# mfkiwl/msckf_stereo_c

Measured on AMD Instinct MI355X. Metric: stereo frames/sec/node on EuRoC-shape input; ATE RMSE vs CPU ref, higher is better.
Workload: dtype f64

## Files before the change

msckf_stereo_c_amd/csrc/hip/fe_kernels.hip:

```cpp
#include <stdlib.h>
#include <mutex>
#include "fe_device.h"

__device__ __forceinline__ int reflect101(int i, int n) {
    if (n == 1) return 0;
    while (i < 0 || i >= n) { i = (i < 0) ? -i : 2 * (n - 1) - i; }
    return i;
}

#define P3_TW 16
#define P3_TH 8
struct Pyr3Job { const uint8_t *src; uint8_t *d1, *d2, *d3; int w0, h0; };

namespace {
constexpr int P3_R2H = 2 * P3_TH + 4, P3_R1H = 2 * P3_R2H + 4, P3_R0H = 2 * P3_R1H + 4;
constexpr int P3_P2W = 2 * P3_TW + 8, P3_P1W = 2 * (2 * P3_TW + 4) + 8;
constexpr int P3_P1S = P3_P1W + 8, P3_P2S = P3_P2W + 8;
typedef uint32_t __attribute__((aligned(1))) pd_u32u;

__device__ __forceinline__ uint2 pd_h4(uint32_t w0, uint32_t w1, uint32_t w2) {
    const int b0 = w0 & 255u, b1 = (w0 >> 8) & 255u, b2 = (w0 >> 16) & 255u, b3 = w0 >> 24, b4 = w1 & 255u, b5 = (w1 >> 8) & 255u,
              b6 = (w1 >> 16) & 255u, b7 = w1 >> 24, b8 = w2 & 255u, b9 = (w2 >> 8) & 255u, b10 = (w2 >> 16) & 255u;
    const uint32_t h0 = (uint32_t)(b0 + 4 * b1 + 6 * b2 + 4 * b3 + b4), h1 = (uint32_t)(b2 + 4 * b3 + 6 * b4 + 4 * b5 + b6);
    const uint32_t h2 = (uint32_t)(b4 + 4 * b5 + 6 * b6 + 4 * b7 + b8), h3 = (uint32_t)(b6 + 4 * b7 + 6 * b8 + 4 * b9 + b10);
// ... 278 lines not shown
    DetPix l_mid = load(ys - 4), l_dn = load(ys - 3), l_nx = load(ys - 2);
    int cy = ys / ch, yin = ys - cy * ch;
    int bs[4] = {0, 0, 0, 0};
    unsigned long long bk[4] = {0ULL, 0ULL, 0ULL, 0ULL};
    const int n_rows = seg_rows;
#pragma unroll 1
    for (int k = 0; k < n_rows; ++k) {
        const int y = ys + k;
        const bool row_ok = y < y_end;
        const DetPix enx = load(pr + 3), lnx = load(y - 1);
        {
            int Ha[4], Hb[4], Hc[4];
            det_hrow(e_up, e_mid, e_dn.hi, Ha, Hb, Hc);
#pragma unroll
            for (int j = 0; j < 4; ++j) { Va[j] += Ha[j]; Vb[j] += Hb[j]; Vc[j] += Hc[j]; }
            e_up = e_mid.hi; e_mid = e_dn; e_dn = e_nx; e_nx = enx; ++pr;
        }
#pragma unroll
        for (int j = 0; j < 4; ++j) {
            if (!(col_ok[j] && row_ok)) continue;
            const int a = Va[j], b = Vb[j], d = Vc[j];
            const int X = (a + d) - max(det_floor, bs[j]);
            if (X <= 0) continue;
            const int df = a - d;
            if (abs(df) >= X || 2 * abs(b) >= X) continue;
            const double discd = (double)df * (double)df + 4.0 * ((double)b * (double)b);
            if (discd >= (double)X * (double)X) continue;
            const long long disc = (long long)df * df + 4LL * ((long long)b * b);
            const int score = (a + d) - (int)isqrt48((unsigned long long)disc, discd);
            bs[j] = score;
            bk[j] = det_key(gen, score, (unsigned int)(yin * cw + xin[j]));
        }
        {
            int Ha[4], Hb[4], Hc[4];
            det_hrow(l_up, l_mid, l_dn.hi, Ha, Hb, Hc);
#pragma unroll
            for (int j = 0; j < 4; ++j) { Va[j] -= Ha[j]; Vb[j] -= Hb[j]; Vc[j] -= Hc[j]; }
            l_up = l_mid.hi; l_mid = l_dn; l_dn = l_nx; l_nx = lnx;
        }
        ++yin;
        const bool flush = job_on && row_ok && (yin == ch || y + 1 == y_end);
        if (cw < 4) {
            if (flush) {
#pragma unroll
                for (int j = 0; j < 4; ++j) {
                    if (bk[j]) atomicMax(&cell_keys[cy * det_cols + cx[j]], bk[j]);
                    bs[j] = 0; bk[j] = 0ULL;
                }
            }
        } else if (__any(flush)) {
            unsigned long long ka = 0ULL, kb = 0ULL;
#pragma unroll
            for (int j = 0; j < 4; ++j) {
                const unsigned long long v = flush ? bk[j] : 0ULL;
                if (cx[j] == cx[0]) ka = v > ka ? v : ka; else kb = v > kb ? v : kb;
            }
            const bool two = cx[3] != cx[0];
#pragma unroll 1
            for (int pass = 0; pass < 2; ++pass) {
                unsigned long long kk = pass ? kb : ka;
                const int id = flush ? (pass ? (two ? cx[3] : -1 - r) : cx[0]) : -1 - r;
                if (pass && !__any(flush && two)) break;
                {
                    const int o = det_dpp0<0x101>(id + 0x40000000) - 0x40000000; const unsigned long long v = det_dpp0_64<0x101>(kk);
                    if (o == id && v > kk) kk = v;
                }
                {
                    const int o = det_dpp0<0x102>(id + 0x40000000) - 0x40000000; const unsigned long long v = det_dpp0_64<0x102>(kk);
                    if (o == id && v > kk) kk = v;
                }
                {
                    const int o = det_dpp0<0x104>(id + 0x40000000) - 0x40000000; const unsigned long long v = det_dpp0_64<0x104>(kk);
                    if (o == id && v > kk) kk = v;
                }
                {
                    const int o = det_dpp0<0x108>(id + 0x40000000) - 0x40000000; const unsigned long long v = det_dpp0_64<0x108>(kk);
                    if (o == id && v > kk) kk = v;
                }
                const int left = det_dpp0<0x111>(id + 0x40000000) - 0x40000000;
                if (id >= 0 && left != id && kk) atomicMax(&cell_keys[cy * det_cols + id], kk);
            }
            if (flush) {
#pragma unroll
                for (int j = 0; j < 4; ++j) { bs[j] = 0; bk[j] = 0ULL; }
            }
        }
        if (yin == ch) { yin = 0; ++cy; }
    }
}

extern "C" void fe_launch_detect(const FeStreamDev *streams_dev, int n_streams, int max_w, int max_h, unsigned int gen, hipStream_t st) {
    const int strips = (max_w - 2 * DET_BORDER + DS_COLS - 1) / DS_COLS, rows = max_h - 2 * DET_BORDER;
    if (strips <= 0 || rows <= 0) return;
    int seg_rows = 32;
    while (seg_rows < 128 && (long long)n_streams * strips * ((rows + seg_rows - 1) / seg_rows) / 4 > 32768) seg_rows *= 2;
    const int segs = (rows + seg_rows - 1) / seg_rows;
    const int waves = (strips * segs + 3) / 4;
    hipLaunchKernelGGL(k_detect_cells, dim3(8 * ((n_streams + 7) / 8) * waves), dim3(64), 0, st, streams_dev, n_streams, strips, seg_rows, waves, gen);
}


__device__ __forceinline__ double det_atan(double x) {
    const bool inv = x > 1.0;
    if (inv) x = 1.0 / x;
    double c = 0.0, ac = 0.0;
    if (x > 0.875)      { c = 1.0;  ac = 0.78539816339744830962; }
    else if (x > 0.625) { c = 0.75; ac = 0.64350110879328438680; }
    else if (x > 0.375) { c = 0.5;  ac = 0.46364760900080611621; }
    else if (x > 0.125) { c = 0.25; ac = 0.24497866312686415417; }
    const double z = (x - c) / (1.0 + x * c);
    const double z2 = z * z;
    double p = 1.0 / 21.0;
    p = 1.0 / 19.0 - z2 * p;
    p = 1.0 / 17.0 - z2 * p;
    p = 1.0 / 15.0 - z2 * p;
    p = 1.0 / 13.0 - z2 * p;
    p = 1.0 / 11.0 - z2 * p;
    p = 1.0 / 9.0 - z2 * p;
    p = 1.0 / 7.0 - z2 * p;
    p = 1.0 / 5.0 - z2 * p;
    p = 1.0 / 3.0 - z2 * p;
    p = 1.0 - z2 * p;
    const double a = ac + z * p;
    return inv ? 1.5707963267948966192 - a : a;
}
__device__ __forceinline__ double det_tan(double t) {
    const bool inv = t > 0.78539816339744830962;
    if (inv) t = 1.5707963267948966192 - t;
    const double t2 = t * t;
    double s = 1.0 / 121645100408832000.0;
    s = 1.0 / 355687428096000.0 - t2 * s;
    s = 1.0 / 1307674368000.0 - t2 * s;
    s = 1.0 / 6227020800.0 - t2 * s;
    s = 1.0 / 39916800.0 - t2 * s;
    s = 1.0 / 362880.0 - t2 * s;
    s = 1.0 / 5040.0 - t2 * s;
    s = 1.0 / 120.0 - t2 * s;
    s = 1.0 / 6.0 - t2 * s;
    s = t * (1.0 - t2 * s);
    double c = 1.0 / 6402373705728000.0;
    c = 1.0 / 20922789888000.0 - t2 * c;
    c = 1.0 / 87178291200.0 - t2 * c;
    c = 1.0 / 479001600.0 - t2 * c;
    c = 1.0 / 3628800.0 - t2 * c;
    c = 1.0 / 40320.0 - t2 * c;
    c = 1.0 / 720.0 - t2 * c;
    c = 1.0 / 24.0 - t2 * c;
    c = 0.5 - t2 * c;
    c = 1.0 - t2 * c;
    return inv ? c / s : s / c;
}


__device__ __forceinline__ void undistort_pt(const CamDev &cam, const double *R, float u, float v, float &xo, float &yo) {
    const double fx = cam.K[0], fy = cam.K[1], cx = cam.K[2], cy = cam.K[3];
    double x = ((double)u - cx) / fx, y = ((double)v - cy) / fy;
    if (cam.model == MSKF_MODEL_EQUIDISTANT) {
        const double *k = cam.D;
        double theta_d = sqrt(x * x + y * y);
        const double half_pi = 1.5707963267948966;
        theta_d = theta_d > half_pi ? half_pi : (theta_d < -half_pi ? -half_pi : theta_d);
        double scale = 0.0;
        if (theta_d > 1e-8) {
            double theta = theta_d;
            for (int j = 0; j < 10; ++j) {
                const double t2 = theta * theta, t4 = t2 * t2, t6 = t4 * t2, t8 = t6 * t2;
                const double k0t2 = k[0] * t2, k1t4 = k[1] * t4, k2t6 = k[2] * t6, k3t8 = k[3] * t8;
                const double fix = (theta * (1 + k0t2 + k1t4 + k2t6 + k3t8) - theta_d) /
                                   (1 + 3 * k0t2 + 5 * k1t4 + 7 * k2t6 + 9 * k3t8);
                theta = theta - fix;
                if (fabs(fix) < 1e-8) break;
            }
            scale = det_tan(theta) / theta_d;
        }
        x = x * scale; y = y * scale;
    } else {
        const double k1 = cam.D[0], k2 = cam.D[1], p1 = cam.D[2], p2 = cam.D[3];
        const double x0 = x, y0 = y;
        for (int j = 0; j < 5; ++j) {
            const double r2 = x * x + y * y;
            const double icdist = 1.0 / (1.0 + (k2 * r2 + k1) * r2);
            const double deltaX = 2.0 * p1 * x * y + p2 * (r2 + 2.0 * x * x);
            const double deltaY = p1 * (r2 + 2.0 * y * y) + 2.0 * p2 * x * y;
            x = (x0 - deltaX) * icdist;
            y = (y0 - deltaY) * icdist;
        }
    }
    if (R) {
        const double X = R[0] * x + R[1] * y + R[2];
        const double Y = R[3] * x + R[4] * y + R[5];
        const double Wd = R[6] * x + R[7] * y + R[8];
        x = X / Wd; y = Y / Wd;
    } else {
        x = x / 1.0; y = y / 1.0;
    }
    xo = (float)(x * 1.0 + 0.0);
    yo = (float)(y * 1.0 + 0.0);
}

__device__ __forceinline__ void distort_pt(const CamDev &cam, float xf, float yf, float &uo, float &vo) {
    const double fx = cam.K[0], fy = cam.K[1], cx = cam.K[2], cy = cam.K[3];
    const double x = (double)xf, y = (double)yf;
    double xd, yd;
    if (cam.model == MSKF_MODEL_EQUIDISTANT) {
        const double *k = cam.D;
        const double r = sqrt(x * x + y * y);
        const double theta = det_atan(r);
        const double t2 = theta * theta, t4 = t2 * t2, t6 = t4 * t2, t8 = t4 * t4;
        const double theta_d = theta * (1 + k[0] * t2 + k[1] * t4 + k[2] * t6 + k[3] * t8);
        const double scale = (r > 1e-8) ? theta_d / r : 1.0;
        xd = x * scale; yd = y * scale;
    } else {
        const double k1 = cam.D[0], k2 = cam.D[1], p1 = cam.D[2], p2 = cam.D[3];
        const double r2 = x * x + y * y, r4 = r2 * r2;
        const double a1 = 2.0 * x * y, a2 = r2 + 2.0 * x * x, a3 = r2 + 2.0 * y * y;
        const double cdist = 1.0 + k1 * r2 + k2 * r4;
        xd = x * cdist + p1 * a1 + p2 * a2;
        yd = y * cdist + p1 * a3 + p2 * a1;
    }
    uo = (float)(xd * fx + cx);
    vo = (float)(yd * fy + cy);
}

#define LK_HALF 7
#define LK_WIN 15
#define LK_ITERS 30

template <int CTRL> __device__ __forceinline__ int dpp_add(int v) {
    return v + __builtin_amdgcn_update_dpp(0, v, CTRL, 0xf, 0xf, false);
}
__device__ __forceinline__ double lk_scaled_f64(long long b) {
    return __longlong_as_double(b + 0x41F8000000000000LL) - 6442450944.0;
}

typedef short l4_v2s __attribute__((ext_vector_type(2)));
#define L4_DW 6
#define L4_TROWS 18
#define L4_SROWS 20
#define L4_MAXOX 8
#define L4_MAXOY (L4_SROWS - 16)

typedef unsigned short l4_v2u __attribute__((ext_vector_type(2)));
template <int KA, int KC> __device__ __forceinline__ int l4_mad24_k(int x) {
    int d;
    asm("v_mad_i32_i24 %0, %1, %2, %3" : "=v"(d) : "n"(KA), "v"(x), "n"(KC));
    return d;
}
template <int KA> __device__ __forceinline__ int l4_mad24_kv(int x, int c) {
    int d;
    asm("v_mad_i32_i24 %0, %1, %2, %3" : "=v"(d) : "n"(KA), "v"(x), "v"(c));
    return d;
}
__device__ __forceinline__ int l4_mad24(int a, int b, int c) {
    int d;
    asm("v_mad_i32_i24 %0, %1, %2, %3" : "=v"(d) : "v"(a), "v"(b), "s"(c));
    return d;
}
__device__ __forceinline__ int l4_mad24_vvv(int a, int b, int c) {
    int d;
    asm("v_mad_i32_i24 %0, %1, %2, %3" : "=v"(d) : "v"(a), "v"(b), "v"(c));
    return d;
}
__device__ __forceinline__ int l4_dot2(int pair, int w, int acc) {
    return __builtin_amdgcn_sdot2(__builtin_bit_cast(l4_v2s, pair), __builtin_bit_cast(l4_v2s, w), acc, false);
}
__device__ __forceinline__ int l4_dot2k(int pair, int w, int k) {
    return __builtin_amdgcn_sdot2(__builtin_bit_cast(l4_v2s, pair), __builtin_bit_cast(l4_v2s, w), k, true);
}
__device__ __forceinline__ int l4_pack_shr9(int a, int b) {
    const l4_v2u v = __builtin_bit_cast(l4_v2u, __builtin_amdgcn_perm((uint32_t)b, (uint32_t)a, 0x06050201u));
    return __builtin_bit_cast(int, (l4_v2u)(v >> (unsigned short)1));
}
#define L4_SHL1 0x101
#define L4_SHR1 0x111
template <int CTRL> __device__ __forceinline__ int l4_dpp0(int v) {
    return __builtin_amdgcn_update_dpp(0, v, CTRL, 0xf, 0xf, true);
}
__device__ __forceinline__ long long l4_row_sum(int v) {
    v = dpp_add<0xB1>(v);
    v = dpp_add<0x4E>(v);
    long long s = (long long)v;
    {
        const int lo = __builtin_amdgcn_update_dpp(0, (int)s, 0x141, 0xf, 0xf, true), hi = __builtin_amdgcn_update_dpp(0, (int)(s >> 32), 0x141, 0xf, 0xf, true);
        s += (long long)(((unsigned long long)(unsigned int)hi << 32) | (unsigned int)lo);
    }
    {
        const int lo = __builtin_amdgcn_update_dpp(0, (int)s, 0x140, 0xf, 0xf, true), hi = __builtin_amdgcn_update_dpp(0, (int)(s >> 32), 0x140, 0xf, 0xf, true);
        s += (long long)(((unsigned long long)(unsigned int)hi << 32) | (unsigned int)lo);
    }
    return s;
}

struct __attribute__((packed, aligned(4))) l4_u4 { uint32_t v[4]; };
struct __attribute__((packed, aligned(4))) l4_u2 { uint32_t v[2]; };
template <int ROWS>
__device__ __forceinline__ void l4_stage(const uint8_t *img, int w, int h, int x0, int y0, uint32_t *dst, int r, bool on) {
    const bool fast = x0 >= 0 && y0 >= 0 && x0 + 4 * L4_DW <= w && y0 + ROWS <= h;
    if (fast) {
        if (on) {
            const uint8_t *p = img + l4_mad24_vvv(y0 + r, w, x0);
            const l4_u4 a = *(const l4_u4 *)p;
            const l4_u2 b = *(const l4_u2 *)(p + 16);
            uint32_t *d = dst + L4_DW * r;
            d[0] = a.v[0]; d[1] = a.v[1]; d[2] = a.v[2]; d[3] = a.v[3]; d[4] = b.v[0]; d[5] = b.v[1];
            if (r < ROWS - 16) {
                const uint8_t *p2 = img + l4_mad24_vvv(y0 + 16 + r, w, x0);
                const l4_u4 a2 = *(const l4_u4 *)p2;
                const l4_u2 b2 = *(const l4_u2 *)(p2 + 16);
                uint32_t *d2 = dst + L4_DW * (16 + r);
                d2[0] = a2.v[0]; d2[1] = a2.v[1]; d2[2] = a2.v[2]; d2[3] = a2.v[3]; d2[4] = b2.v[0]; d2[5] = b2.v[1];
            }
        }
        return;
    }
    constexpr int N = ROWS * L4_DW, PER = (N + 15) / 16;
    typedef uint32_t __attribute__((aligned(1))) l4_u32u;
    uint32_t v[PER];
#pragma unroll
    for (int i = 0; i < PER; ++i) {
        const int e = r + 16 * i;
        v[i] = 0;
        if (on && e < N) {
            const int row = (e * 43) >> 8, c = e - L4_DW * row;
            const uint8_t *rp = img + l4_mad24_vvv(min(max(y0 + row, 0), h - 1), w, 0);
            const int xb = x0 + 4 * c, xc = min(max(xb, 0), w - 4), sh = xb - xc;
            const uint32_t D = *(const l4_u32u *)(rp + xc);
            const uint32_t first = (D & 255u) * 0x01010101u, last = (D >> 24) * 0x01010101u;
            v[i] = sh < 0 ? first : sh >= 4 ? last : __builtin_amdgcn_alignbyte(last, D, (uint32_t)sh);
        }
    }
#pragma unroll
    for (int i = 0; i < PER; ++i) { const int e = r + 16 * i; if (on && e < N) dst[e] = v[i]; }
}

template <int K> __device__ __forceinline__ int l4_pair(const uint32_t *a) {
    constexpr int q = K >> 2, m = K & 3;
    if (m == 0) return (int)__builtin_amdgcn_perm(0u, a[q], 0x0c010c00u);
    if (m == 1) return (int)__builtin_amdgcn_perm(0u, a[q], 0x0c020c01u);
    if (m == 2) return (int)__builtin_amdgcn_perm(0u, a[q], 0x0c030c02u);
    return (int)__builtin_amdgcn_perm(a[q + 1], a[q], 0x0c040c03u);
}
template <int N, int K = 0> struct L4Pairs {
    static __device__ __forceinline__ void run(const uint32_t *a, int *pr) { pr[K] = l4_pair<K>(a); L4Pairs<N, K + 1>::run(a, pr); }
};
template <int N> struct L4Pairs<N, N> { static __device__ __forceinline__ void run(const uint32_t *, int *) {} };

__device__ __forceinline__ void l4_weights(float fa, float fb, int &wtop, int &wbot) {
    const int qa = __float2int_rn(fa * 16384.0f), qb = __float2int_rn(fb * 16384.0f);
    const int w00 = l4_mad24(16384 - qa, 16384 - qb, 8192) >> 14;
    const int w01 = l4_mad24(qa, 16384 - qb, 8192) >> 14;
// ... 15 lines not shown
        const float sc = __int_as_float((127 - l) << 23);
        const float pwx = ax * sc - (float)LK_HALF, pwy = ay * sc - (float)LK_HALF;
        if (l == MSKF_LEVELS - 1) { ncx = bx * sc; ncy = by * sc; }
        else { ncx = ncx * 2.0f; ncy = ncy * 2.0f; }
        int ipx = (int)floorf(pwx), ipy = (int)floorf(pwy);
        bool lvl_on = alive && !(ipx < -LK_WIN || ipx >= aw || ipy < -LK_WIN || ipy >= ah);
        if (alive && !lvl_on && l == 0) status = 0;
        if (!lvl_on) { ipx = 0; ipy = 0; }
        int wtop, wbot;
        l4_weights(lvl_on ? pwx - (float)ipx : 0.f, lvl_on ? pwy - (float)ipy : 0.f, wtop, wbot);
        const int ax0 = (ipx - 1) & ~3, ay0 = ipy - 1, oxa = ipx - 1 - ax0;
        float wx = ncx - (float)LK_HALF, wy = ncy - (float)LK_HALF;
        int inx0 = (int)floorf(wx), iny0 = (int)floorf(wy);
        const bool in_b0 = !(inx0 < -LK_WIN || inx0 >= bw || iny0 < -LK_WIN || iny0 >= bh);
        if (!(lvl_on && in_b0)) { inx0 = 0; iny0 = 0; }
        int bx0 = (inx0 - 2) & ~3, by0 = iny0 - 2;
        __syncthreads();
        l4_stage<L4_TROWS>(imA, aw, ah, ax0, ay0, sT, r, true);
        l4_stage<L4_SROWS>(imB, bw, bh, bx0, by0, sS, r, true);
        __syncthreads();
        int V[17], E[17];
        {
            uint32_t d[6], a[5];
            int pr[17];
            const uint32_t *rp = sT + (r + 1) * L4_DW;
#pragma unroll
            for (int i = 0; i < 6; ++i) d[i] = rp[i];
#pragma unroll
            for (int i = 0; i < 5; ++i) a[i] = __builtin_amdgcn_alignbyte(d[i + 1], d[i], oxa);
            L4Pairs<17>::run(a, pr);
            int Bv[17];
#pragma unroll
            for (int c = 0; c < 17; ++c) { V[c] = l4_dot2k(pr[c], wtop, 256); Bv[c] = l4_dot2k(pr[c], wbot, 0); }
            const uint32_t *ep = sT + (r == 0 ? 0 : 17) * L4_DW;
#pragma unroll
            for (int i = 0; i < 6; ++i) d[i] = ep[i];
#pragma unroll
            for (int i = 0; i < 5; ++i) a[i] = __builtin_amdgcn_alignbyte(d[i + 1], d[i], oxa);
            L4Pairs<17>::run(a, pr);
            const int wsel = r == 0 ? wtop : wbot;
#pragma unroll
            for (int c = 0; c < 17; ++c) E[c] = l4_dot2(pr[c], wsel, r == 0 ? Bv[c] + 256 : V[c]) >> 9;
#pragma unroll
            for (int c = 0; c < 17; ++c) V[c] = (V[c] + l4_dpp0<L4_SHL1>(Bv[c])) >> 9;
            if (r == 15) {
#pragma unroll
                for (int c = 0; c < 17; ++c) V[c] = E[c];
            }
        }
        int Pp[8], Ixp[8], Iyp[8];
        int A11 = 0, A12 = 0, A22 = 0;
        {
            int f[17], e[17];
#pragma unroll
            for (int c = 0; c < 17; ++c) {
                const int up = __builtin_amdgcn_update_dpp(E[c], V[c], L4_SHR1, 0xf, 0xf, false);
                const int dn = l4_dpp0<L4_SHL1>(V[c]);
                f[c] = up + dn; e[c] = dn - up;
            }
            int gx[16], gy[16], pv[16];
#pragma unroll
            for (int i = 0; i < 15; ++i) {
                const int sx = l4_mad24_kv<10>(V[i + 2] - V[i], l4_mad24_k<3, 16>(f[i + 2] - f[i]));
                const int sy = l4_mad24_kv<10>(e[i + 1], l4_mad24_k<3, 16>(e[i] + e[i + 2]));
                gx[i] = sx >> 5;
                gy[i] = sy >> 5;
                pv[i] = V[i + 1];
            }
            gx[15] = 0; gy[15] = 0; pv[15] = 0;
#pragma unroll
            for (int m = 0; m < 8; ++m) {
                const int ix = (int)__builtin_amdgcn_perm((uint32_t)gx[2 * m + 1], (uint32_t)gx[2 * m], 0x05040100u);
                const int iy = (int)__builtin_amdgcn_perm((uint32_t)gy[2 * m + 1], (uint32_t)gy[2 * m], 0x05040100u);
                Ixp[m] = winrow ? ix : 0;
                Iyp[m] = winrow ? iy : 0;
                Pp[m] = (int)__builtin_amdgcn_perm((uint32_t)pv[2 * m + 1], (uint32_t)pv[2 * m], 0x05040100u);
                A11 = l4_dot2(Ixp[m], Ixp[m], A11); A12 = l4_dot2(Ixp[m], Iyp[m], A12); A22 = l4_dot2(Iyp[m], Iyp[m], A22);
            }
        }
        const long long A11s = l4_row_sum(A11), A12s = l4_row_sum(A12), A22s = l4_row_sum(A22);
        const double a11 = lk_scaled_f64(A11s), a12 = lk_scaled_f64(A12s), a22 = lk_scaled_f64(A22s);
        double D = a11 * a22 - a12 * a12;
        const double dd = a11 - a22;
        const double numer = a22 + a11 - sqrt(dd * dd + 4.0 * a12 * a12);
        bool run = lvl_on && !(numer < 0x1.70a3d70a3d70bp-5 || D < 1.1920928955078125e-07);
        if (lvl_on && !run && l == 0) status = 0;
        const bool solved = run;
        D = 1.0 / D;
        float pdx = 0.f, pdy = 0.f;
        for (int it = 0; it < LK_ITERS; ++it) {
            if (!__any(run)) break;
#ifdef LK_ITER_DBG
            if (run) dbg_iters += 1u << (8 * l);
#endif
            int inx = (int)floorf(wx), iny = (int)floorf(wy);
            if (run && (inx < -LK_WIN || inx >= bw || iny < -LK_WIN || iny >= bh)) {
                if (l == 0) status = 0;
                run = false;
            }
            int ox = inx - bx0, oy = iny - by0;
            const bool need = run && (ox < 0 || ox > L4_MAXOX || oy < 0 || oy > L4_MAXOY);
            if (__any(need)) {
                if (need) { bx0 = (inx - 2) & ~3; by0 = iny - 2; }
                __syncthreads();
                l4_stage<L4_SROWS>(imB, bw, bh, bx0, by0, sS, r, need);
                __syncthreads();
                ox = inx - bx0; oy = iny - by0;
            }
            if (!run) { ox = 0; oy = 0; }
            int wt, wb;
            l4_weights(wx - (float)inx, wy - (float)iny, wt, wb);
            uint32_t d[5], a[4];
            const uint32_t *rp = sS + l4_mad24_kv<L4_DW>(oy + r, ox >> 2);
#pragma unroll
            for (int i = 0; i < 5; ++i) d[i] = rp[i];
#pragma unroll
            for (int i = 0; i < 4; ++i) a[i] = __builtin_amdgcn_alignbyte(d[i + 1], d[i], ox & 3);
            int pr[15];
            L4Pairs<15>::run(a, pr);
            int sv[16];
#pragma unroll
            for (int k = 0; k < 15; ++k) {
                const int t = l4_dot2k(pr[k], wt, 256), b = l4_dot2k(pr[k], wb, 0);
                sv[k] = t + l4_dpp0<L4_SHL1>(b);
            }
            sv[15] = 0;
            int b1 = 0, b2 = 0;
#pragma unroll
            for (int m = 0; m < 8; ++m) {
                const l4_v2s sp = __builtin_bit_cast(l4_v2s, l4_pack_shr9(sv[2 * m], sv[2 * m + 1]));
                const int df = __builtin_bit_cast(int, (l4_v2s)(sp - __builtin_bit_cast(l4_v2s, Pp[m])));
                b1 = l4_dot2(df, Ixp[m], b1);
                b2 = l4_dot2(df, Iyp[m], b2);
            }
            const long long b1s = l4_row_sum(b1), b2s = l4_row_sum(b2);
            const double db1 = lk_scaled_f64(b1s), db2 = lk_scaled_f64(b2s);
            const float dx = (float)((a12 * db2 - a22 * db1) * D);
            const float dy = (float)((a12 * db1 - a11 * db2) * D);
            if (run) {
                wx += dx; wy += dy;
                if ((double)dx * (double)dx + (double)dy * (double)dy <= 1e-4) run = false;
                else if (it > 0 && fabsf(dx + pdx) < 0.01f && fabsf(dy + pdy) < 0.01f) {
                    wx -= dx * 0.5f; wy -= dy * 0.5f;
                    run = false;
                }
                pdx = dx; pdy = dy;
            }
        }
        if (solved) { ncx = wx + (float)LK_HALF; ncy = wy + (float)LK_HALF; }
    }
    out_x = ncx; out_y = ncy; out_status = status;
}

__global__ __launch_bounds__(64) void k_track4(const FeStreamDev *streams, int n_streams, int groups_per_stream) {
    const int x = blockIdx.x & 7, qb = blockIdx.x >> 3;
    const int si = x + 8 * (qb / groups_per_stream), gi = qb - (qb / groups_per_stream) * groups_per_stream;
    if (si >= n_streams) return;
    const FeStreamDev &S = streams[si];
    const int n_pts = S.n_pts_dev ? *S.n_pts_dev : S.n_pts;
    const int lane = threadIdx.x & 63, g = lane >> 4, r = lane & 15;
    __shared__ uint32_t s_T[4][L4_TROWS * L4_DW + 2];
    __shared__ uint32_t s_S[4][L4_SROWS * L4_DW + 4];
    uint32_t *sT = s_T[g], *sS = s_S[g];
#pragma nounroll
    for (int gq = gi; 4 * gq < n_pts; gq += groups_per_stream) {
    const int pt = 4 * gq + g;
    const bool in_range = pt < n_pts;
    mskf_point2f pin = {0.f, 0.f};
    if (in_range) pin = S.in_pts[pt];
    unsigned int dbg_iters = 0, dbg_t = 0;
    float c0x = pin.x, c0y = pin.y;
    bool ok = in_range;
    float tx = 0.f, ty = 0.f, gx = 0.f, gy = 0.f;
    bool alive = false;
    int ph = 1;
    if (S.do_temporal) {
        const double *Hm = S.Hpred;
        const double px = (double)pin.x, py = (double)pin.y;
        const double X = Hm[0] * px + Hm[1] * py + Hm[2] * 1.0;
        const double Y = Hm[3] * px + Hm[4] * py + Hm[5] * 1.0;
        const double Z = Hm[6] * px + Hm[7] * py + Hm[8] * 1.0;
        tx = pin.x; ty = pin.y; gx = (float)(X / Z); gy = (float)(Y / Z);
        alive = in_range;
        ph = 0;
    }
    float c1x = 0.f, c1y = 0.f;
    int st1 = 0;
#pragma nounroll
    for (; ph < 2; ++ph) {
        if (ph == 1) {
            gx = 0.f; gy = 0.f;
            if (ok) {
                float rx, ry;
                undistort_pt(S.cam0, S.R01, c0x, c0y, rx, ry);
                distort_pt(S.cam1, rx, ry, gx, gy);
            }
            tx = c0x; ty = c0y; alive = ok;
        }
        float nx = 0.f, ny = 0.f;
        int st = 0;
        if (__any(alive)) l4_track(ph ? S.curr0 : S.prev0, ph ? S.curr1 : S.curr0, alive, tx, ty, gx, gy, sT, sS, r, nx, ny, st, dbg_iters);
        if (ph == 0) {
            const int W = S.curr0.w[0], H = S.curr0.h[0];
            c0x = nx; c0y = ny;
            ok = alive && st != 0 && !(c0y < 0 || c0y > (float)(H - 1) || c0x < 0 || c0x > (float)(W - 1));
            dbg_t = dbg_iters; dbg_iters = 0;
        } else {
            c1x = alive ? nx : 0.f; c1y = alive ? ny : 0.f; st1 = alive ? st : 0;
        }
    }
    float u0x = 0.f, u0y = 0.f, u1x = 0.f, u1y = 0.f;
    int sst = st1;
    if (ok) {
        const int W1 = S.curr1.w[0], H1 = S.curr1.h[0];
        if (sst && (c1y < 0 || c1y > (float)(H1 - 1) || c1x < 0 || c1x > (float)(W1 - 1))) sst = 0;
        undistort_pt(S.cam0, nullptr, c0x, c0y, u0x, u0y);
        undistort_pt(S.cam1, nullptr, c1x, c1y, u1x, u1y);
        if (sst) {
            const double *E = S.E;
            const double x0 = (double)u0x, y0 = (double)u0y, x1 = (double)u1x, y1 = (double)u1y;
            const double l0 = (E[0] * x0 + E[1] * y0) + E[2];
            const double l1 = (E[3] * x0 + E[4] * y0) + E[5];
            const double l2 = (E[6] * x0 + E[7] * y0) + E[8];
            const double err = fabs((x1 * l0 + y1 * l1) + l2) / sqrt(l0 * l0 + l1 * l1);
            if (err > S.epi_thresh) sst = 0;
        }
    }
    if (in_range && r == 0) {
        S.out0[pt] = mskf_point2f{c0x, c0y};
        S.out1[pt] = mskf_point2f{c1x, c1y};
        S.und0[pt] = mskf_point2f{u0x, u0y};
#ifdef LK_ITER_DBG
        ((unsigned int *)S.und1)[2 * pt] = dbg_t; ((unsigned int *)S.und1)[2 * pt + 1] = dbg_iters;
#else
        S.und1[pt] = mskf_point2f{u1x, u1y};
        (void)dbg_t;
#endif
        S.status[pt] = (uint8_t)(ok ? (1 | (sst ? 2 : 0)) : 0);
    }
    }
}

#include "fe_book.h"
__global__ __launch_bounds__(256) void k_fe_book(const FeBookDev *books, int which) {
    const FeBookDev &B = books[blockIdx.x];
    extern __shared__ int s_book[];
    FeBookScratch L;
    fe_book_scratch_init(L, s_book, B.cap, B.cand_cap, B.det_cap, B.n_codes, B.det_rows * B.det_cols);
    if (which == 0) fe_book1(B, L); else fe_book2(B, L);
}
extern "C" size_t fe_book_lds_budget(void) {
    static const size_t budget = []() -> size_t {
        const hipError_t e = hipFuncSetAttribute(reinterpret_cast<const void *>(k_fe_book), hipFuncAttributeMaxDynamicSharedMemorySize, 150 * 1024);
        if (e != hipSuccess) { (void)hipGetLastError(); return 64 * 1024; }
        return 150 * 1024;
    }();
    return budget;
}
extern "C" void fe_launch_book(const FeBookDev *books_dev, int n_streams, int which, size_t scratch_bytes, hipStream_t st) {
    (void)fe_book_lds_budget();
    hipLaunchKernelGGL(k_fe_book, dim3(n_streams), dim3(256), scratch_bytes, st, books_dev, which);
}

#include "fe_equalize.h"
namespace {
struct __attribute__((packed, aligned(1))) eq_u4 { uint32_t v[4]; };
__device__ __forceinline__ int eq_block_scan(int v, int *s, int tid) {
    s[tid] = v;
    __syncthreads();
    for (int off = 1; off < 256; off <<= 1) {
        const int t = tid >= off ? s[tid - off] : 0;
        __syncthreads();
        s[tid] += t;
        __syncthreads();
    }
    return s[tid];
}
__device__ __forceinline__ void eq_count16(int *hw, const uint32_t v[4], int lo, int hi) {
#pragma unroll
    for (int k = 0; k < 16; ++k)
        if (k >= lo && k < hi) atomicAdd(&hw[(v[k >> 2] >> (8 * (k & 3))) & 255u], 1);
}
}

__global__ __launch_bounds__(256) void k_eq_hist(const EqJob *jobs) {
    const EqJob j = jobs[blockIdx.y];
    const int unit = blockIdx.x, tid = threadIdx.x;
    const int n_units = j.mode == EQ_CLAHE ? j.tiles_x * j.tiles_y : j.n_strips;
    if (unit >= n_units) return;
    __shared__ int s_hist[4][256];
    __shared__ int s_scan[256];
#pragma unroll
    for (int k = 0; k < 4; ++k) s_hist[k][tid] = 0;
    __syncthreads();
    int r0, r1, c0, c1;
    if (j.mode == EQ_CLAHE) {
        const int ty = unit / j.tiles_x, tx = unit - ty * j.tiles_x;
        r0 = ty * j.th; r1 = r0 + j.th; c0 = tx * j.tw; c1 = c0 + j.tw;
    } else {
        r0 = unit * j.strip_rows; r1 = min(j.h, r0 + j.strip_rows); c0 = 0; c1 = j.w;
    }
    int *hw = s_hist[tid >> 6];
    const int w = j.w, h = j.h, cr = min(c1, w);
    if (cr > c0) {
        const uintptr_t img_b = (uintptr_t)j.src, img_e = img_b + (size_t)w * h;
        const int nch = (cr - c0 + 15) / 16 + 1;
        const int n_items = (r1 - r0) * nch;
        for (int idx = tid; idx < n_items; idx += 256) {
            const int rr = idx / nch, ch = idx - rr * nch;
            const uintptr_t a = img_b + (size_t)eq_src_row(r0 + rr, h) * w + c0, e = a + (size_t)(cr - c0);
            const uintptr_t q = (a & ~(uintptr_t)15) + 16 * (uintptr_t)ch;
            if (q >= e) continue;
            const int lo = a > q ? (int)(a - q) : 0, hi = e - q < 16 ? (int)(e - q) : 16;
            if (q >= img_b && q + 16 <= img_e) {
                const uint4 v = *reinterpret_cast<const uint4 *>(q);
                const uint32_t vv[4] = {v.x, v.y, v.z, v.w};
                eq_count16(hw, vv, lo, hi);
            } else {
                for (int k = lo; k < hi; ++k) atomicAdd(&hw[*reinterpret_cast<const uint8_t *>(q + k)], 1);
            }
        }
    }
    if (c1 > w) {
        const int cv0 = max(c0, w), nv = c1 - cv0, n_items = (r1 - r0) * nv;
        for (int idx = tid; idx < n_items; idx += 256) {
            const int rr = idx / nv, c = cv0 + idx - rr * nv;
            atomicAdd(&hw[j.src[(size_t)eq_src_row(r0 + rr, h) * w + eq_src_col(c, w)]], 1);
        }
    }
    __syncthreads();
    const int cnt = s_hist[0][tid] + s_hist[1][tid] + s_hist[2][tid] + s_hist[3][tid];
    if (j.mode != EQ_CLAHE) { j.part[256 * unit + tid] = cnt; return; }
    (void)eq_block_scan(eq_excess(cnt, j.clip), s_scan, tid);
    const int clipped = s_scan[255];
    __syncthreads();
    const int cum = eq_block_scan(eq_redistributed(cnt, tid, j.clip, clipped), s_scan, tid);
    j.lut[256 * (size_t)unit + tid] = (uint8_t)eq_clahe_entry(cum, eq_clahe_scale(j.tw * j.th));
}

__global__ __launch_bounds__(256) void k_eq_lut(const EqJob *jobs) {
    const EqJob j = jobs[blockIdx.x];
    if (j.mode != EQ_GLOBAL) return;
    const int tid = threadIdx.x;
    __shared__ int s_scan[256], s_cnt[256], s_i0;
    int cnt = 0;
    for (int s = 0; s < j.n_strips; ++s) cnt += j.part[256 * s + tid];
    s_cnt[tid] = cnt;
    if (tid == 0) s_i0 = 255;
    __syncthreads();
    if (cnt > 0) atomicMin(&s_i0, tid);
    const int cum = eq_block_scan(cnt, s_scan, tid);
    const int i0 = s_i0;
    j.lut[tid] = (uint8_t)eq_global_entry(tid, i0, s_cnt[i0], cum, j.w * j.h);
}

__global__ __launch_bounds__(256) void k_eq_apply(const EqJob *jobs, int splits) {
    const EqJob j = jobs[blockIdx.y];
    const int region = blockIdx.x / splits, split = blockIdx.x - region * splits, tid = threadIdx.x;
    if (region >= eq_regions(j.mode, j.tiles_x, j.tiles_y)) return;
    const bool clahe = j.mode == EQ_CLAHE;
    const int w = j.w, h = j.h;
    int x0 = 0, x1 = w, y0 = 0, y1 = h, t1x = 0, t2x = 0, t1y = 0, t2y = 0;
    float inv_tw = 0.f, inv_th = 0.f;
    if (clahe) {
        const int nrx = j.tiles_x + 1, ry = region / nrx, rx = region - ry * nrx;
        inv_tw = eq_inv(j.tw); inv_th = eq_inv(j.th);
        x0 = rx == 0 ? 0 : eq_axis_first(rx - 1, j.tw, inv_tw, w); x1 = rx == j.tiles_x ? w : eq_axis_first(rx, j.tw, inv_tw, w);
        y0 = ry == 0 ? 0 : eq_axis_first(ry - 1, j.th, inv_th, h); y1 = ry == j.tiles_y ? h : eq_axis_first(ry, j.th, inv_th, h);
        t1x = max(rx - 1, 0); t2x = min(rx, j.tiles_x - 1); t1y = max(ry - 1, 0); t2y = min(ry, j.tiles_y - 1);
    }
    const int rp = (y1 - y0 + splits - 1) / splits, ya = y0 + split * rp, yb = min(y1, ya + rp);
    if (ya >= yb || x0 >= x1) return;
    __shared__ uint32_t s_lut[256];
    if (clahe) {
        const uint8_t *r1 = j.lut + 256 * (size_t)(t1y * j.tiles_x), *r2 = j.lut + 256 * (size_t)(t2y * j.tiles_x);
        s_lut[tid] = (uint32_t)r1[256 * t1x + tid] | ((uint32_t)r1[256 * t2x + tid] << 8) | ((uint32_t)r2[256 * t1x + tid] << 16) | ((uint32_t)r2[256 * t2x + tid] << 24);
    } else s_lut[tid] = j.lut[tid];
    __syncthreads();
    const int nch = (x1 - x0 + 15) / 16 + 1, n_items = (yb - ya) * nch;
    for (int idx = tid; idx < n_items; idx += 256) {
        const int rr = idx / nch, ch = idx - rr * nch, y = ya + rr;
        const size_t row = (size_t)y * w, pb = row + x0, pe = row + x1;
        const size_t P = (pb & ~(size_t)15) + 16 * (size_t)ch;
        if (P >= pe) continue;
        const int lo = pb > P ? (int)(pb - P) : 0, hi = pe - P < 16 ? (int)(pe - P) : 16;
        const bool whole = lo == 0 && hi == 16;
        uint32_t in[4] = {0u, 0u, 0u, 0u}, out[4] = {0u, 0u, 0u, 0u};
        if (whole) { const eq_u4 v = *reinterpret_cast<const eq_u4 *>(j.src + P); in[0] = v.v[0]; in[1] = v.v[1]; in[2] = v.v[2]; in[3] = v.v[3]; }
        else {
// ... 18 lines not shown
#pragma unroll
            for (int k = 0; k < 16; ++k) if (k >= lo && k < hi) j.dst[P + k] = (uint8_t)(out[k >> 2] >> (8 * (k & 3)));
        }
    }
}

extern "C" void fe_launch_equalize(const EqJob *jobs_dev, int n_jobs, int max_units, int any_global, int max_regions, int splits, hipStream_t st) {
    if (n_jobs <= 0) return;
    hipLaunchKernelGGL(k_eq_hist, dim3(max_units, n_jobs), dim3(256), 0, st, jobs_dev);
    if (any_global) hipLaunchKernelGGL(k_eq_lut, dim3(n_jobs), dim3(256), 0, st, jobs_dev);
    hipLaunchKernelGGL(k_eq_apply, dim3(max_regions * splits, n_jobs), dim3(256), 0, st, jobs_dev, splits);
}

#include "fe_pixfmt.h"
namespace {
#if defined(__HIP_DEVICE_COMPILE__)
#define PX_GLOBAL __attribute__((address_space(1)))
#else
#define PX_GLOBAL
#endif
typedef const PX_GLOBAL uint8_t *px_gptr;
__device__ __forceinline__ px_gptr px_global(const uint8_t *p) { return (px_gptr)(uintptr_t)p; }
__device__ __forceinline__ uint32_t px_byte(const uint32_t *v, int i) { return (v[i >> 2] >> (8 * (i & 3))) & 255u; }
template <int NV>
__device__ __forceinline__ void px_load(uint32_t *v, px_gptr p) {
#pragma unroll
    for (int q = 0; q < NV; ++q) {
        const eq_u4 t = *reinterpret_cast<const PX_GLOBAL eq_u4 *>(p + 16 * q);
        v[4 * q] = t.v[0]; v[4 * q + 1] = t.v[1]; v[4 * q + 2] = t.v[2]; v[4 * q + 3] = t.v[3];
    }
}
template <int FMT>
__device__ __forceinline__ void px_chunk16(const PxJob &j, int x0, int y, uint32_t out[4]) {
    out[0] = out[1] = out[2] = out[3] = 0u;
    constexpr int BPP = FMT == PX_GRAY16 ? 2 : (FMT == PX_RGB8 || FMT == PX_BGR8) ? 3 : 4;
    uint32_t v[4 * BPP];
    px_load<BPP>(v, px_global(j.src) + (size_t)y * (size_t)j.pitch + (size_t)x0 * BPP);
#pragma unroll
    for (int k = 0; k < 16; ++k) {
        int g;
        if (FMT == PX_GRAY16) g = px_gray16((int)((v[k >> 1] >> (16 * (k & 1))) & 0xFFFFu), j.shift);
        else {
            const int c0 = (int)px_byte(v, BPP * k), c1 = (int)px_byte(v, BPP * k + 1), c2 = (int)px_byte(v, BPP * k + 2);
            g = (FMT == PX_RGB8 || FMT == PX_RGBA8) ? px_luma(c0, c1, c2) : px_luma(c2, c1, c0);
        }
        out[k >> 2] |= (uint32_t)g << (8 * (k & 3));
    }
}
__device__ __forceinline__ void px_chunk16_bayer(const PxJob &j, int x0, int y, uint32_t out[4]) {
    out[0] = out[1] = out[2] = out[3] = 0u;
    const px_gptr src = px_global(j.src);
    const px_gptr rows[3] = {src + (size_t)px_reflect(y - 1, j.h) * (size_t)j.pitch + x0, src + (size_t)y * (size_t)j.pitch + x0,
                             src + (size_t)px_reflect(y + 1, j.h) * (size_t)j.pitch + x0};
    uint32_t v[3][4], lft[3], rgt[3];
#pragma unroll
    for (int r = 0; r < 3; ++r) { px_load<1>(v[r], rows[r]); lft[r] = rows[r][-1]; rgt[r] = rows[r][16]; }
    const int site0 = px_bayer_site(j.format, x0, y), site1 = px_bayer_site(j.format, x0 + 1, y);
#pragma unroll
    for (int k = 0; k < 16; ++k) {
        int a[3], b[3], c[3];
#pragma unroll
        for (int r = 0; r < 3; ++r) {
            a[r] = (int)(k == 0 ? lft[r] : px_byte(v[r], k - 1));
            b[r] = (int)px_byte(v[r], k);
            c[r] = (int)(k == 15 ? rgt[r] : px_byte(v[r], k + 1));
        }
        const int g = px_bayer_luma((k & 1) ? site1 : site0, b[1], a[1], c[1], b[0], b[2], a[0], c[0], a[2], c[2]);
        out[k >> 2] |= (uint32_t)g << (8 * (k & 3));
    }
}
template <int FMT>
__device__ __forceinline__ void px_rows(const PxJob &j) {
    const int w = j.w, h = j.h;
    const int nch = (w + 15) / 16 + 1;
    const long long n_items = (long long)h * nch;
    for (long long idx = (long long)blockIdx.x * 256 + threadIdx.x; idx < n_items; idx += (long long)gridDim.x * 256) {
        const int y = (int)(idx / nch), ch = (int)(idx - (long long)y * nch);
        const uintptr_t pb = (uintptr_t)j.dst + (size_t)y * w, pe = pb + (size_t)w;
        const uintptr_t P = (pb & ~(uintptr_t)15) + 16 * (uintptr_t)ch;
        if (P >= pe) continue;
        const int lo = pb > P ? (int)(pb - P) : 0, hi = pe - P < 16 ? (int)(pe - P) : 16;
        const int x0 = (int)((long long)P - (long long)pb);
        bool whole = lo == 0 && hi == 16;
        if (FMT == PX_BAYER_RGGB8) whole = whole && x0 >= 1 && x0 + 16 <= w - 1;
        if (whole) {
            uint32_t out[4];
            if (FMT == PX_BAYER_RGGB8) px_chunk16_bayer(j, x0, y, out); else px_chunk16<FMT>(j, x0, y, out);
            *reinterpret_cast<PX_GLOBAL uint4 *>(P) = make_uint4(out[0], out[1], out[2], out[3]);
        } else {
            for (int k = lo; k < hi; ++k) *reinterpret_cast<PX_GLOBAL uint8_t *>(P + k) = (uint8_t)px_pixel(j.src, (size_t)j.pitch, w, h, j.format, j.shift, x0 + k, y);
        }
    }
}
}

__global__ __launch_bounds__(256) void k_px_convert(const PxJob *jobs) {
    const PxJob j = jobs[blockIdx.y];
    switch (j.format) {
        case PX_GRAY16: px_rows<PX_GRAY16>(j); break;
        case PX_RGB8: px_rows<PX_RGB8>(j); break;
        case PX_BGR8: px_rows<PX_BGR8>(j); break;
        case PX_RGBA8: px_rows<PX_RGBA8>(j); break;
        case PX_BGRA8: px_rows<PX_BGRA8>(j); break;
        case PX_BAYER_RGGB8: case PX_BAYER_GRBG8: case PX_BAYER_GBRG8: case PX_BAYER_BGGR8: px_rows<PX_BAYER_RGGB8>(j); break;
        default: break;
    }
}

extern "C" void fe_launch_px_convert(const PxJob *jobs_dev, int n_jobs, int max_w, int max_h, hipStream_t st) {
    if (n_jobs <= 0 || max_w <= 0 || max_h <= 0) return;
    const long long items = (long long)max_h * ((max_w + 15) / 16 + 1);
    const long long wgs = (items + 255) / 256;
    hipLaunchKernelGGL(k_px_convert, dim3((unsigned)(wgs > 65535 ? 65535 : wgs), n_jobs), dim3(256), 0, st, jobs_dev);
}

__global__ void k_mark(volatile unsigned int *flag, unsigned int seq) {
    *flag = seq;
    __threadfence_system();
}
extern "C" void fe_launch_mark(volatile unsigned int *flag, unsigned int seq, hipStream_t st) {
    hipLaunchKernelGGL(k_mark, dim3(1), dim3(1), 0, st, flag, seq);
}

struct MskfCopySegs { void *dst[MSKF_COPY_SEGS]; const void *src[MSKF_COPY_SEGS]; unsigned long long bytes[MSKF_COPY_SEGS]; int blocks_per_seg; };
__global__ __launch_bounds__(256) void k_mskf_copy(MskfCopySegs segs) {
    const int seg = (int)blockIdx.x / segs.blocks_per_seg, b = (int)blockIdx.x - seg * segs.blocks_per_seg;
    const unsigned long long bytes = segs.bytes[seg], n16 = bytes >> 4;
    const uint4 *__restrict__ src = (const uint4 *)segs.src[seg];
    uint4 *__restrict__ dst = (uint4 *)segs.dst[seg];
    const unsigned long long stride = (unsigned long long)segs.blocks_per_seg * 256ULL;
    unsigned long long i = (unsigned long long)b * 256ULL + threadIdx.x;
    for (; i + 3ULL * stride < n16; i += 4ULL * stride) {
        const uint4 a0 = src[i], a1 = src[i + stride], a2 = src[i + 2ULL * stride], a3 = src[i + 3ULL * stride];
        dst[i] = a0; dst[i + stride] = a1; dst[i + 2ULL * stride] = a2; dst[i + 3ULL * stride] = a3;
    }
    for (; i < n16; i += stride) dst[i] = src[i];
    if (b == 0 && threadIdx.x < (unsigned)(bytes & 15ULL)) ((uint8_t *)dst)[(n16 << 4) + threadIdx.x] = ((const uint8_t *)src)[(n16 << 4) + threadIdx.x];
}
extern "C" void fe_launch_copy(void *const *dst, const void *const *src, const size_t *bytes, int n_segs, hipStream_t st) {
    MskfCopySegs segs;
    size_t mx = 0;
    for (int i = 0; i < MSKF_COPY_SEGS; ++i) {
        segs.dst[i] = i < n_segs ? dst[i] : nullptr; segs.src[i] = i < n_segs ? src[i] : nullptr; segs.bytes[i] = i < n_segs ? bytes[i] : 0ULL;
        if (i < n_segs && bytes[i] > mx) mx = bytes[i];
    }
    if (n_segs <= 0 || mx == 0) return;
    size_t bps = (mx + 16383) / 16384;
    segs.blocks_per_seg = (int)(bps < 1 ? 1 : bps > 96 ? 96 : bps);
    hipLaunchKernelGGL(k_mskf_copy, dim3(segs.blocks_per_seg * n_segs), dim3(256), 0, st, segs);
}

extern "C" void fe_launch_track(const FeStreamDev *streams_dev, int n_streams, int max_pts, hipStream_t st) {
    if (max_pts <= 0) return;
    const int gps = (max_pts + 3) / 4;
    hipLaunchKernelGGL(k_track4, dim3(8 * ((n_streams + 7) / 8) * gps), dim3(64), 0, st, streams_dev, n_streams, gps);
}
```

Baseline: 102,500.

## Parallelize per-point undistort/distort across lanes and reuse cam0 undistortion

Restructures the LK tracking kernel so each lane owns one point for the scalar camera math (homography, undistort, distort, epipolar check), with per-point state staged in shared memory. Previously all 16 lanes of a group redundantly computed the same point's math. The 16-lane groups then loop over the points, running l4_track from the shared state. The cam0 undistortion result from the stereo phase is reused instead of being recomputed. This adds block barriers and shared-memory traffic. With the default TRK_PTS=4 only 4 lanes do the scalar work, and the barriers may cost more than the redundancy saved.

```diff
diff --git a/msckf_stereo_c_amd/csrc/hip/fe_kernels.hip b/msckf_stereo_c_amd/csrc/hip/fe_kernels.hip
--- a/msckf_stereo_c_amd/csrc/hip/fe_kernels.hip
+++ b/msckf_stereo_c_amd/csrc/hip/fe_kernels.hip
@@ -454,7 +454,7 @@
 }
 
 
-__device__ __forceinline__ void undistort_pt(const CamDev &cam, const double *R, float u, float v, float &xo, float &yo) {
+__device__ __forceinline__ void undistort_core(const CamDev &cam, float u, float v, double &xn, double &yn) {
     const double fx = cam.K[0], fy = cam.K[1], cx = cam.K[2], cy = cam.K[3];
     double x = ((double)u - cx) / fx, y = ((double)v - cy) / fy;
     if (cam.model == MSKF_MODEL_EQUIDISTANT) {
@@ -488,6 +488,9 @@
             y = (y0 - deltaY) * icdist;
         }
     }
+    xn = x; yn = y;
+}
+__device__ __forceinline__ void undistort_finish(const double *R, double x, double y, float &xo, float &yo) {
     if (R) {
         const double X = R[0] * x + R[1] * y + R[2];
         const double Y = R[3] * x + R[4] * y + R[5];
@@ -498,6 +501,11 @@
     }
     xo = (float)(x * 1.0 + 0.0);
     yo = (float)(y * 1.0 + 0.0);
+}
+__device__ __forceinline__ void undistort_pt(const CamDev &cam, const double *R, float u, float v, float &xo, float &yo) {
+    double x, y;
+    undistort_core(cam, u, v, x, y);
+    undistort_finish(R, x, y, xo, yo);
 }
 
 __device__ __forceinline__ void distort_pt(const CamDev &cam, float xf, float yf, float &uo, float &vo) {
@@ -819,69 +827,93 @@
     out_x = ncx; out_y = ncy; out_status = status;
 }
 
+#ifndef TRK_PTS
+#define TRK_PTS 4
+#endif
+static_assert(TRK_PTS == 4 || TRK_PTS == 8 || TRK_PTS == 16, "TRK_PTS: 4, 8 or 16");
+enum { TRK_ALIVE, TRK_TX, TRK_TY, TRK_GX, TRK_GY, TRK_NX, TRK_NY, TRK_ST, TRK_DBG, TRK_DBGT, TRK_FIELDS };
+
 __global__ __launch_bounds__(64) void k_track4(const FeStreamDev *streams, int n_streams, int groups_per_stream) {
     const int x = blockIdx.x & 7, qb = blockIdx.x >> 3;
     const int si = x + 8 * (qb / groups_per_stream), gi = qb - (qb / groups_per_stream) * groups_per_stream;
     if (si >= n_streams) return;
     const FeStreamDev &S = streams[si];
     const int n_pts = S.n_pts_dev ? *S.n_pts_dev : S.n_pts;
-    const int lane = threadIdx.x & 63, g = lane >> 4, r = lane & 15;
+    const int lane = threadIdx.x & 63, g = lane >> 4, r = lane & 15, pl = lane & (TRK_PTS - 1);
     __shared__ uint32_t s_T[4][L4_TROWS * L4_DW + 2];
     __shared__ uint32_t s_S[4][L4_SROWS * L4_DW + 4];
+    __shared__ float s_pt[TRK_FIELDS][TRK_PTS];
+    __shared__ double s_n0[2][TRK_PTS];
     uint32_t *sT = s_T[g], *sS = s_S[g];
 #pragma nounroll
-    for (int gq = gi; 4 * gq < n_pts; gq += groups_per_stream) {
-    const int pt = 4 * gq + g;
-    const bool in_range = pt < n_pts;
-    mskf_point2f pin = {0.f, 0.f};
-    if (in_range) pin = S.in_pts[pt];
-    unsigned int dbg_iters = 0, dbg_t = 0;
-    float c0x = pin.x, c0y = pin.y;
-    bool ok = in_range;
-    float tx = 0.f, ty = 0.f, gx = 0.f, gy = 0.f;
-    bool alive = false;
+    for (int gq = gi; TRK_PTS * gq < n_pts; gq += groups_per_stream) {
+    const int pt = TRK_PTS * gq + pl;
+    const bool in_range = pt < n_pts, writer = lane < TRK_PTS;
     int ph = 1;
-    if (S.do_temporal) {
-        const double *Hm = S.Hpred;
-        const double px = (double)pin.x, py = (double)pin.y;
-        const double X = Hm[0] * px + Hm[1] * py + Hm[2] * 1.0;
-        const double Y = Hm[3] * px + Hm[4] * py + Hm[5] * 1.0;
-        const double Z = Hm[6] * px + Hm[7] * py + Hm[8] * 1.0;
-        tx = pin.x; ty = pin.y; gx = (float)(X / Z); gy = (float)(Y / Z);
-        alive = in_range;
-        ph = 0;
-    }
-    float c1x = 0.f, c1y = 0.f;
-    int st1 = 0;
+    {
+        mskf_point2f pin = {0.f, 0.f};
+        if (in_range) pin = S.in_pts[pt];
+        float gx = 0.f, gy = 0.f;
+        if (S.do_temporal) {
+            const double *Hm = S.Hpred;
+            const double px = (double)pin.x, py = (double)pin.y;
+            const double X = Hm[0] * px + Hm[1] * py + Hm[2] * 1.0;
+            const double Y = Hm[3] * px + Hm[4] * py + Hm[5] * 1.0;
+            const double Z = Hm[6] * px + Hm[7] * py + Hm[8] * 1.0;
+            gx = (float)(X / Z); gy = (float)(Y / Z);
+            ph = 0;
+        }
+        if (writer) {
+            s_pt[TRK_ALIVE][pl] = in_range ? 1.f : 0.f; s_pt[TRK_TX][pl] = pin.x; s_pt[TRK_TY][pl] = pin.y; s_pt[TRK_GX][pl] = gx; s_pt[TRK_GY][pl] = gy;
+            s_pt[TRK_DBGT][pl] = 0.f; s_n0[0][pl] = 0.0; s_n0[1][pl] = 0.0;
+        }
+    }
 #pragma nounroll
     for (; ph < 2; ++ph) {
         if (ph == 1) {
-            gx = 0.f; gy = 0.f;
-            if (ok) {
+            const float c0x = s_pt[TRK_TX][pl], c0y = s_pt[TRK_TY][pl];
+            float gx = 0.f, gy = 0.f;
+            double n0x = 0.0, n0y = 0.0;
+            if (s_pt[TRK_ALIVE][pl] != 0.f) {
                 float rx, ry;
-                undistort_pt(S.cam0, S.R01, c0x, c0y, rx, ry);
+                undistort_core(S.cam0, c0x, c0y, n0x, n0y);
+                undistort_finish(S.R01, n0x, n0y, rx, ry);
                 distort_pt(S.cam1, rx, ry, gx, gy);
             }
-            tx = c0x; ty = c0y; alive = ok;
-        }
-        float nx = 0.f, ny = 0.f;
-        int st = 0;
-        if (__any(alive)) l4_track(ph ? S.curr0 : S.prev0, ph ? S.curr1 : S.curr0, alive, tx, ty, gx, gy, sT, sS, r, nx, ny, st, dbg_iters);
+            if (writer) { s_pt[TRK_GX][pl] = gx; s_pt[TRK_GY][pl] = gy; s_n0[0][pl] = n0x; s_n0[1][pl] = n0y; }
+        }
+        if (writer) { s_pt[TRK_NX][pl] = 0.f; s_pt[TRK_NY][pl] = 0.f; s_pt[TRK_ST][pl] = 0.f; s_pt[TRK_DBG][pl] = 0.f; }
+        __syncthreads();
+#pragma nounroll
+        for (int j = 0; j < TRK_PTS / 4; ++j) {
+            const int q = 4 * j + g;
+            const bool s_alive = s_pt[TRK_ALIVE][q] != 0.f;
+            if (!__any(s_alive)) continue;
+            float s_nx = 0.f, s_ny = 0.f;
+            int s_st = 0;
+            unsigned int s_dbg = 0;
+            l4_track(ph ? S.curr0 : S.prev0, ph ? S.curr1 : S.curr0, s_alive, s_pt[TRK_TX][q], s_pt[TRK_TY][q], s_pt[TRK_GX][q], s_pt[TRK_GY][q],
+                     sT, sS, r, s_nx, s_ny, s_st, s_dbg);
+            if (r == 0) { s_pt[TRK_NX][q] = s_nx; s_pt[TRK_NY][q] = s_ny; s_pt[TRK_ST][q] = (float)s_st; s_pt[TRK_DBG][q] = __uint_as_float(s_dbg); }
+        }
+        __syncthreads();
         if (ph == 0) {
             const int W = S.curr0.w[0], H = S.curr0.h[0];
-            c0x = nx; c0y = ny;
-            ok = alive && st != 0 && !(c0y < 0 || c0y > (float)(H - 1) || c0x < 0 || c0x > (float)(W - 1));
-            dbg_t = dbg_iters; dbg_iters = 0;
-        } else {
-            c1x = alive ? nx : 0.f; c1y = alive ? ny : 0.f; st1 = alive ? st : 0;
-        }
-    }
+            const float c0x = s_pt[TRK_NX][pl], c0y = s_pt[TRK_NY][pl];
+            const bool ok = s_pt[TRK_ALIVE][pl] != 0.f && s_pt[TRK_ST][pl] != 0.f && !(c0y < 0 || c0y > (float)(H - 1) || c0x < 0 || c0x > (float)(W - 1));
+            const float dbg = s_pt[TRK_DBG][pl];
+            if (writer) { s_pt[TRK_TX][pl] = c0x; s_pt[TRK_TY][pl] = c0y; s_pt[TRK_ALIVE][pl] = ok ? 1.f : 0.f; s_pt[TRK_DBGT][pl] = dbg; }
+        }
+    }
+    const float c0x = s_pt[TRK_TX][pl], c0y = s_pt[TRK_TY][pl];
+    const bool ok = s_pt[TRK_ALIVE][pl] != 0.f;
+    const float c1x = ok ? s_pt[TRK_NX][pl] : 0.f, c1y = ok ? s_pt[TRK_NY][pl] : 0.f;
     float u0x = 0.f, u0y = 0.f, u1x = 0.f, u1y = 0.f;
-    int sst = st1;
+    int sst = ok ? (int)s_pt[TRK_ST][pl] : 0;
     if (ok) {
         const int W1 = S.curr1.w[0], H1 = S.curr1.h[0];
         if (sst && (c1y < 0 || c1y > (float)(H1 - 1) || c1x < 0 || c1x > (float)(W1 - 1))) sst = 0;
-        undistort_pt(S.cam0, nullptr, c0x, c0y, u0x, u0y);
+        undistort_finish(nullptr, s_n0[0][pl], s_n0[1][pl], u0x, u0y);
         undistort_pt(S.cam1, nullptr, c1x, c1y, u1x, u1y);
         if (sst) {
             const double *E = S.E;
@@ -893,15 +925,14 @@
             if (err > S.epi_thresh) sst = 0;
         }
     }
-    if (in_range && r == 0) {
+    if (in_range && lane < TRK_PTS) {
         S.out0[pt] = mskf_point2f{c0x, c0y};
         S.out1[pt] = mskf_point2f{c1x, c1y};
         S.und0[pt] = mskf_point2f{u0x, u0y};
 #ifdef LK_ITER_DBG
-        ((unsigned int *)S.und1)[2 * pt] = dbg_t; ((unsigned int *)S.und1)[2 * pt + 1] = dbg_iters;
+        ((unsigned int *)S.und1)[2 * pt] = __float_as_uint(s_pt[TRK_DBGT][pl]); ((unsigned int *)S.und1)[2 * pt + 1] = __float_as_uint(s_pt[TRK_DBG][pl]);
 #else
         S.und1[pt] = mskf_point2f{u1x, u1y};
-        (void)dbg_t;
 #endif
         S.status[pt] = (uint8_t)(ok ? (1 | (sst ? 2 : 0)) : 0);
     }
@@ -1226,6 +1257,6 @@
 
 extern "C" void fe_launch_track(const FeStreamDev *streams_dev, int n_streams, int max_pts, hipStream_t st) {
     if (max_pts <= 0) return;
-    const int gps = (max_pts + 3) / 4;
+    const int gps = (max_pts + TRK_PTS - 1) / TRK_PTS;
     hipLaunchKernelGGL(k_track4, dim3(8 * ((n_streams + 7) / 8) * gps), dim3(64), 0, st, streams_dev, n_streams, gps);
 }
```

Result: slower. 98240 (-4.2%).
